# thu-ml/SageAttention

Measured on AMD Instinct MI355X. Metric: attention TFLOPS (causal, hd=128), kernel-only, as published by the reference, higher is better.
Workload: dtype int8 QK^T + fp8(e4m3) PV, fp32 accumulate

## Files before the change

sageattention_amd/csrc/sage_attn.hip:

```cpp
#include "sage_common.h"
#include "sage_kernels.h"
#include "sage_attn_parts.h"
#include "sage_work_order.h"
#include <cstdlib>

#ifndef SAGE_ORDER_DEFAULT
#define SAGE_ORDER_DEFAULT -1
#endif

namespace sage {

static int g_work_order = -2;
int work_order()
{
    if (g_work_order == -2) {
        const char *e = getenv("SAGE_ORDER_GROUP");
        g_work_order = (e != nullptr && e[0] != 0) ? atoi(e) : SAGE_ORDER_DEFAULT;
    }
    return g_work_order;
}
void set_work_order_mode(int group) { g_work_order = group; }

static int plan_grid(AttnParams &q, const AttnVariant &v)
{
    q.order_group = 0;
    q.order_fold = 0;
    q.order_left = 0;
    const int nheads = q.B * q.Hq;
    if (q.cu_q != nullptr && q.work_items != nullptr)
        return 8 * ((q.Hq & 7) * ((q.items_bound + 7) / 8) + (q.Hq >> 3) * q.items_bound);
    if (q.cu_q != nullptr) return ((q.B * q.Hkv + 7) / 8) * 8 * q.group * q.nqblk;
    const int forced = work_order();
    if (!v.causal || v.mask_kind != 0 || v.seeded || q.kv_split > 1 || q.nqblk <= 1 || forced == 0) return nheads * q.nqblk;
    WorkOrder w;
    const int grid = plan_work_order(w, nheads, q.nqblk, q.Lk, v.head_dim, v.pv_fp8, forced);
    q.order_group = w.group;
    q.order_fold = w.fold;
    q.order_left = w.left;
    return grid;
}

static bool route_exists(const AttnParams &p, const AttnVariant &v, const AttnLaunchOpts &o)
{
    const bool varlen = p.cu_q != nullptr, per_thread = v.qf == 1 || v.qf == 2, per_block = v.qf == 3 || v.qf == 4;
    if ((v.head_dim != 64 && v.head_dim != 128) || v.qf < 0 || v.qf > 4 || v.mask_kind < 0 || v.mask_kind > 3) return false;
    if (v.mask_kind != 0 && (v.qf != 0 || v.pv_fp8 || v.causal || v.kthread || !v.two_level)) return false;
    if (per_thread && (varlen || !v.kthread || v.two_level != v.pv_fp8)) return false;
    if (per_block && (v.kthread || (v.pv_fp8 ? (!varlen || o.fp8_folded) : !v.two_level))) return false;
    if (p.v_rows != 0 && (v.pv_fp8 || v.mask_kind != 0 || varlen || p.kv_split > 1 || v.qf == 2 || v.qf == 4)) return false;
    if ((v.seeded || v.kv_lens) && (!per_thread || !v.pv_fp8 || o.fp8_folded || (v.seeded && v.kv_lens))) return false;
    if (v.seeded != (p.seed_max != nullptr) || (v.seeded && p.kv_split < 1)) return false;
    if (v.kv_lens && (p.cu_k == nullptr || p.kv_split > 1)) return false;
    if (v.q_start != (!varlen && p.cu_qs != nullptr) || (v.q_start && (!v.kv_lens || !v.causal))) return false;
    return true;
}

hipError_t launch_attention(const AttnParams &p_in, const AttnVariant &v, const AttnLaunchOpts &o)
{
    AttnParams p = p_in;
    const int nwork = plan_grid(p, v);
    if (o.grid_out != nullptr) *o.grid_out = 0;
    if (nwork <= 0) return hipSuccess;
    if (!route_exists(p, v, o)) return hipErrorInvalidValue;
    const bool d128 = v.head_dim == 128;
    if (v.seeded) return d128 ? launch_attn_f8_seeded<128>(p, v, nwork, o) : launch_attn_f8_seeded<64>(p, v, nwork, o);
    if (v.q_start) return d128 ? launch_attn_f8_qstart<128>(p, v, nwork, o) : launch_attn_f8_qstart<64>(p, v, nwork, o);
    if (v.kv_lens) return d128 ? launch_attn_f8_kvlens<128>(p, v, nwork, o) : launch_attn_f8_kvlens<64>(p, v, nwork, o);
    if (v.pv_fp8 && v.qf >= 3) return d128 ? launch_attn_f8_varlen<128>(p, v, nwork, o) : launch_attn_f8_varlen<64>(p, v, nwork, o);
    if (!v.pv_fp8) return d128 ? launch_attn_part<128, false, true>(p, v, nwork, o) : launch_attn_part<64, false, true>(p, v, nwork, o);
    if (o.fp8_folded) return d128 ? launch_attn_part<128, true, true>(p, v, nwork, o) : launch_attn_part<64, true, true>(p, v, nwork, o);
    return d128 ? launch_attn_part<128, true, false>(p, v, nwork, o) : launch_attn_part<64, true, false>(p, v, nwork, o);
}

}
```

sageattention_amd/csrc/sage_attn_kernel.h:

```cpp
#pragma once
#include "sage_common.h"
#include "sage_kernels.h"
#include "sage_attn_parts.h"
#include "sage_quant_math.h"
#include "sage_work_order.h"
#include <atomic>
#include <climits>
#include <cstdlib>
#include <type_traits>

#ifndef SAGE_ABL
#define SAGE_ABL 0
#endif
#ifndef SAGE_DIAG_PIPE
#define SAGE_DIAG_PIPE 1
#endif
#ifndef SAGE_KARG_PREFETCH
#define SAGE_KARG_PREFETCH 1
#endif
#ifndef SAGE_TAIL_PIPE
#define SAGE_TAIL_PIPE 1
#endif
#ifndef SAGE_KSEL
#define SAGE_KSEL 1
// ... 38 lines not shown
{
    v16i d;
    asm("s_nop 1\n\tv_mfma_i32_32x32x32_i8 %0, %1, %2, 0x3e22f983" : "=&v"(d) : "v"(a), "v"(b));
    return d;
}

#if SAGE_ATTN_TRACE
#define SAGE_TSTAMP(i) do { if (wave == 0) { unsigned long long t_; \
    asm volatile("s_memrealtime %0\n\ts_waitcnt lgkmcnt(0)" : "=s"(t_) :: "memory"); ttrace[i] = (unsigned)t_; } } while (0)
#else
#define SAGE_TSTAMP(i) do { } while (0)
#endif

template <int D, bool PV_FP8, bool CAUSAL, bool KTHREAD, bool TWO_LEVEL, int NH, int MASK = 0, int QF = 0, bool SFOLD = true, bool CPERS = false,
          bool VROWS = false, bool SEED = false, bool QSTART = false, bool KVLEN = false>
__global__ void __launch_bounds__(256, SAGE_MIN_WAVES(D, MASK))
sage_attn_kernel(const AttnParams p_arg)
{
    typedef const __attribute__((address_space(4))) AttnParams *kparams_t;
    const kparams_t kp0 = (kparams_t)__builtin_amdgcn_kernarg_segment_ptr();
    const __attribute__((address_space(4))) AttnParams &p = *kp0;
    (void)p_arg;
#if SAGE_KARG_PREFETCH
    static_assert(sizeof(AttnParams) > 0x180, "prefetch offsets lie inside the parameter block");
    {
        unsigned t0, t1, t2, t3, t4, t5, t6;
        asm volatile("s_load_dword %0, %7, 0x0\n\ts_load_dword %1, %7, 0x40\n\ts_load_dword %2, %7, 0x80\n\ts_load_dword %3, %7, 0xc0\n\t"
                     "s_load_dword %4, %7, 0x100\n\ts_load_dword %5, %7, 0x140\n\ts_load_dword %6, %7, 0x180\n\ts_waitcnt lgkmcnt(0)"
                     : "=&s"(t0), "=&s"(t1), "=&s"(t2), "=&s"(t3), "=&s"(t4), "=&s"(t5), "=&s"(t6) : "s"(kp0) : "memory");
    }
#endif
    using C = TileCfg<D, PV_FP8, NH>;
    constexpr int KT = C::KT;
    constexpr int NS = 2 * NH;
    static_assert(!SEED || (PV_FP8 && KTHREAD && TWO_LEVEL && !SFOLD && MASK == 0 && (QF == 1 || QF == 2) && !CPERS && !VROWS),
                  "the seeded split: FP8 PV, fused per-thread Q, exact score form, dense");
    static_assert(!KVLEN || (PV_FP8 && KTHREAD && TWO_LEVEL && !SFOLD && MASK == 0 && (QF == 1 || QF == 2) && !CPERS && !VROWS && !SEED),
                  "per-sample key lengths: FP8 PV, fused per-thread Q, exact score form, dense");
    static_assert(!QSTART || (KVLEN && CAUSAL), "per-sample query offsets: the causal kv_lens kernels");
    extern __shared__ __attribute__((aligned(16))) unsigned char smem[];

    const int wave_s = __builtin_amdgcn_readfirstlane((int)threadIdx.x >> 6);
#if SAGE_ATTN_TRACE
    __shared__ unsigned ttrace[16];
#endif
    constexpr bool PERS_OK = (!CAUSAL || CPERS) && MASK == 0;
    const bool pers = PERS_OK && p.sched != nullptr;
    __shared__ int s_ticket[2];
    int tpar = 0;
    int bid = blockIdx.x;
    unsigned next_k_v = 0;
    bool have_next = false, own_empty = false;
// ... 38 lines not shown
            if (lane_o == 0) kv = __hip_atomic_fetch_add(sched + 32 * bq, 1u, __ATOMIC_RELAXED, __HIP_MEMORY_SCOPE_AGENT);
            const int i = 32 * ((int)__builtin_amdgcn_readfirstlane(kv) + sched_first) + 8 * (bq & 3) + (bq >> 2);
            if (i < nwg_l) return i;
        }
        return -1;
    };
    while (bid >= 0) {
    next_k_v = 0;
    do {
    kparams_t kp = kp0;
    if constexpr (PERS_OK) asm volatile("" : "+s"(kp));
    const __attribute__((address_space(4))) AttnParams &p = *kp;
    int lane_v = (int)__builtin_amdgcn_mbcnt_hi(~0u, __builtin_amdgcn_mbcnt_lo(~0u, 0u));
    if constexpr (PERS_OK) asm volatile("v_mbcnt_lo_u32_b32 %0, -1, 0\n\tv_mbcnt_hi_u32_b32 %0, -1, %0" : "=v"(lane_v));
    const int lane = lane_v;
    const int wave = wave_s;
    [[maybe_unused]] const int tid = wave * 64 + lane;
    int n = lane & 31;
    int g = lane >> 5;
    SAGE_TSTAMP(0);
    __builtin_amdgcn_s_setreg(kHwregModeFp16Ovfl, 1);

    const int nqblk = p.nqblk;
    int b, h, hk, qblk;
    if (p.cu_q != nullptr && p.work_items != nullptr) {
        typedef const __attribute__((address_space(4))) int *cint_p;
        const cint_p hdr = (cint_p)p.work_hdr;
        const int nitems = hdr[0];
        const WorkOrder wo = {hdr[1], hdr[2], hdr[3]};
        const int nwg = 8 * (wo.left * ((nitems + 7) >> 3) + (p.Hq >> 3) * nitems);
        int qrank;
        if (bid >= nwg || !work_item(wo, bid, nwg, p.Hq, nitems, h, qrank)) break;
        const cint_p items = (cint_p)p.work_items;
        b = items[2 * qrank];
        qblk = items[2 * qrank + 1];
        hk = h / p.group;
    } else if (p.cu_q != nullptr) {
        const int xcd = bid & 7, idx = bid >> 3;
        const int per_unit = nqblk * p.group;
        const int j = idx / per_unit, within = idx - j * per_unit;
        const int u = j * 8 + xcd;
        if (u >= p.B * p.Hkv) break;
        const int r = within / p.group, hg = within - r * p.group;
        qblk = nqblk - 1 - r;
        const int bs = u / p.Hkv;
        hk = u - bs * p.Hkv;
        b = p.seq_order != nullptr ? p.seq_order[bs] : bs;
        h = hk * p.group + hg;
    } else {
        int bh, qrank;
        const WorkOrder wo = {CAUSAL ? p.order_group : 0, p.order_fold, p.order_left};
        if (!work_item(wo, bid, pers ? p.nwg : (int)gridDim.x, p.B * p.Hq, nqblk, bh, qrank)) break;
        qblk = nqblk - 1 - qrank;
        b = bh / p.Hq;
        h = bh - b * p.Hq;
        hk = h / p.group;
    }

    int Lq = p.Lq, Lk = p.Lk;
    [[maybe_unused]] int qstart = 0;
    long q_off, k_off, o_off;
    long v_tile0, v_tstride;
    const float *qs_ptr, *ks_ptr;
    int qs_stride, ks_tstride;
    if (p.cu_q != nullptr) {
        typedef const __attribute__((address_space(4))) int *cint_p;
        const int bu = __builtin_amdgcn_readfirstlane(b);
        const int q0 = ((cint_p)p.cu_q)[bu], k0 = ((cint_p)p.cu_k)[bu], q1 = ((cint_p)p.cu_q)[bu + 1], k1 = ((cint_p)p.cu_k)[bu + 1];
        const int ks0 = ((cint_p)p.cu_ks)[bu];
        Lq = q1 - q0;
        Lk = k1 - k0;
        if (qblk * BLKQ >= Lq) break;
        q_off = (long)q0 * p.q_sl + (long)h * p.q_sh;
        k_off = (long)k0 * p.k_sl + (long)hk * p.k_sh;
        o_off = (long)q0 * p.o_sl + (long)h * p.o_sh;
        v_tile0 = (long)ks0 * p.Hkv + hk;
        v_tstride = p.Hkv;
        qs_ptr = QF == 0 ? p.q_scale + ((long)((cint_p)p.cu_qs)[bu] + qblk) * p.Hq + h : nullptr;
        qs_stride = 0;
        ks_ptr = p.k_scale + (long)ks0 * p.Hkv + hk;
        ks_tstride = p.Hkv;
    } else if constexpr (SEED) {
        const int hk0 = hk / p.kv_split, kc0 = p.kv_base + (hk - hk0 * p.kv_split) * Lk;
        const long bh0 = (long)b * (p.Hkv / p.kv_split) + hk0;
        q_off = (long)b * p.q_sb + (long)(hk0 * p.group + (h - hk * p.group)) * p.q_sh;
        k_off = (long)b * p.k_sb + (long)hk0 * p.k_sh + (long)kc0 * p.k_sl;
        o_off = (long)b * p.o_sb + (long)h * p.o_sh;
        v_tile0 = bh0 * (p.nks >> 2) + (kc0 >> 6);
        v_tstride = 1;
        qs_ptr = nullptr;
        qs_stride = 0;
        ks_ptr = p.k_scale + bh0 * p.nks + (kc0 >> 6) * 4;
        ks_tstride = 4;
    } else {
        const int hq = p.kv_split > 1 ? (hk / p.kv_split) * p.group + (h - hk * p.group) : h;
        if constexpr (KVLEN) {
            typedef const __attribute__((address_space(4))) int *cint_p;
            const int len = ((cint_p)p.cu_k)[__builtin_amdgcn_readfirstlane(b)];
            Lk = len < 0 ? 0 : (len < p.Lk ? len : p.Lk);
            if constexpr (QSTART) {
                const int s = ((cint_p)p.cu_qs)[__builtin_amdgcn_readfirstlane(b)];
                qstart = s < -p.Lq ? -p.Lq : (s < p.Lk ? s : p.Lk);
            }
        }
        q_off = (long)b * p.q_sb + (long)hq * p.q_sh;
        k_off = (long)b * p.k_sb + (long)hk * p.k_sh;
        o_off = (long)b * p.o_sb + (long)h * p.o_sh;
        const int ntk = ((KVLEN ? p.Lk : Lk) + BLKK - 1) / BLKK;
        v_tile0 = ((long)b * p.Hkv + hk) * ntk;
        v_tstride = 1;
        qs_ptr = p.q_scale + ((long)b * p.Hq + h) * p.nqs + (long)qblk * p.qs_per_blk;
        qs_stride = 1;
        ks_ptr = p.k_scale + ((long)b * p.Hkv + hk) * p.nks;
        ks_tstride = KTHREAD ? 4 : 1;
    }

    SAGE_TSTAMP(1);
    const int row0 = qblk * BLKQ + wave * 32;
    int my_row = row0 + n;
    const int kchunk0 = QSTART ? -qstart
                      : SEED ? (CAUSAL ? p.kv_base + (hk % p.kv_split) * Lk : 0)
                             : ((CAUSAL && p.kv_split > 1 && p.cu_q == nullptr) ? (hk % p.kv_split) * Lk : 0);
    const int crow0 = row0 - kchunk0;
    int cmy_row = my_row - kchunk0;
    const int ntk_all = (Lk + BLKK - 1) / BLKK;
    int n_iters = (Lk + KT - 1) / KT;
    if (CAUSAL) {
        int lim = (qblk * BLKQ + BLKQ - kchunk0 + KT - 1) / KT;
        lim = lim > 0 ? lim : 0;
        n_iters = lim < n_iters ? lim : n_iters;
    }

    v4i qf[C::KSTEPS];
    float qsc;
    const unsigned char *kbase = reinterpret_cast<const unsigned char *>(p.k) + k_off;
    static_assert(!VROWS || (!PV_FP8 && MASK == 0), "V rows in place: FP16 PV, unmasked, dense launches");
    const unsigned char *vbase = reinterpret_cast<const unsigned char *>(p.v) + (VROWS ? 2 * ((long)b * p.v_sb + (long)hk * p.v_sh) : 0L);
    constexpr int CPR = D / 16;
    constexpr int KP = C::K_TILE_BYTES / 1024, VP = C::V_IMG_BYTES / 1024;
    unsigned koff[KP / 4];
#pragma unroll
    for (int i = 0; i < KP / 4; i++) {
        const int e = (wave * (KP / 4) + i) * 64 + lane;
        const int row = e / CPR, phys = e % CPR;
        koff[i] = (unsigned)(row * (int)p.k_sl + swz_chunk<D>(row, phys) * 16);
// ... 168 lines not shown
        amax = fmaxf(amax, __shfl_xor(amax, 32));
        if constexpr (QBLOCK) {
            __shared__ float q_amax[4];
            if (lane == 0) q_amax[wave] = amax;
            asm volatile("s_waitcnt lgkmcnt(0)" ::: "memory");
            __builtin_amdgcn_s_barrier();
            amax = fmaxf(fmaxf(q_amax[0], q_amax[1]), fmaxf(q_amax[2], q_amax[3]));
        }
        const float sc = quant_scale(amax, QBLOCK ? QS_TRITON : QS_TRITON_THREAD);
        const float y = quant_recip(sc);
        qsc = sc;
#pragma unroll
        for (int ks = 0; ks < C::KSTEPS; ks++) {
            int q8[16];
#pragma unroll
            for (int j = 0; j < 16; j++) q8[j] = QBLOCK ? quant_round_triton(x[ks][j], sc, y) : quant_round_triton_nz(x[ks][j], sc, y);
#pragma unroll
            for (int w = 0; w < 4; w++) qf[ks][w] = (int)pack_int8x4(q8[4 * w], q8[4 * w + 1], q8[4 * w + 2], q8[4 * w + 3]);
        }
    }

    if constexpr (SEED) {
        if (my_row < Lq) {
            const int hk0 = hk / p.kv_split;
            const long gl = (long)p.group * Lq;
            const float *sm = p.seed_max + ((long)b * (p.Hkv / p.kv_split) + hk0) * p.seed_chunks * gl + (long)(h - hk * p.group) * Lq + my_row;
            const int c_end = p.seed_first + (hk - hk0 * p.kv_split);
            for (int c = 0; c < c_end; c++) m_run = fmaxf(m_run, sm[c * gl]);
        }
    }
    SAGE_TSTAMP(2);
    ring_wait(n_iters > 1);
    SAGE_TSTAMP(3);

    int cur = 0;
    auto tile_iter = [&](const int it) {
        const bool more = (it + 1) < n_iters;
        const bool more2 = (it + 2) < n_iters;
        const int nxt = (cur + 1 == NSTAGE) ? 0 : cur + 1;
        float ksc_next[NH][2];
        if (more) load_kscales(it + 1, ksc_next);
        if (more2) issue_loads(it + 2, (nxt + 1 == NSTAGE) ? 0 : nxt + 1);

        int nact = 0;
#pragma unroll
        for (int hh = 0; hh < NH; hh++) {
            const int key0 = it * KT + hh * BLKK;
            if (key0 < Lk && (!CAUSAL || key0 <= crow0 + 31)) nact = hh + 1;
        }
// ... 247 lines not shown
        }
    }
    if constexpr (MASK == 0) {
        asm volatile("v_mbcnt_lo_u32_b32 %0, -1, 0\n\tv_mbcnt_hi_u32_b32 %0, -1, %0" : "=v"(lane_g));
        n = lane_g & 31;
        g = lane_g >> 5;
        my_row = row0 + n;
        cmy_row = my_row - kchunk0;
    }
#pragma nounroll
    for (; it < n_iters; it++) tile_iter(it);
    SAGE_TSTAMP(4);
    __syncthreads();
    SAGE_TSTAMP(5);
    if (pers && !own_empty) {
        if (wave == 0 && lane_g == 0) next_k_v = __hip_atomic_fetch_add(kpl()->sched + 32 * my_queue(), 1u, __ATOMIC_RELAXED, __HIP_MEMORY_SCOPE_AGENT);
        have_next = true;
    }

    __builtin_amdgcn_s_setreg(kHwregModeFp16Ovfl, 0);
    const float l_tot = pair_sum(l_run);
    const float inv = l_tot > 0.0f ? __builtin_amdgcn_rcpf(l_tot) : 0.0f;
    if (p.lse != nullptr && g == 0 && my_row < Lq) {
        long lidx = (p.cu_q != nullptr) ? ((long)h * p.lse_sh + p.cu_q[b] + my_row)
                                        : ((long)b * p.Hq + h) * (long)p.Lq + my_row;
        p.lse[lidx] = __builtin_amdgcn_logf(l_tot) + m_run;
    }
    unsigned char *obuf = smem + wave * (32 * D * 2);
    const long vbh = SEED ? (long)b * (p.Hkv / p.kv_split) + hk / p.kv_split : (long)b * p.Hkv + hk;
    const float *vsc = PV_FP8 ? p.v_scale + vbh * D : nullptr;
    const float *vmn = (p.v_mean != nullptr) ? p.v_mean + vbh * D : nullptr;
    v4f sc4[C::DT][4], mn4[C::DT][4];
    [[maybe_unused]] unsigned keep = (!KVLEN || Lk > 0) ? ~0u : 0u;
    if constexpr (KVLEN) asm volatile("" : "+v"(keep));
#pragma unroll
    for (int dt = 0; dt < C::DT; dt++) {
#pragma unroll
        for (int r4 = 0; r4 < 4; r4++) {
            const v4f one = {1.0f, 1.0f, 1.0f, 1.0f};
            sc4[dt][r4] = PV_FP8 ? *reinterpret_cast<const v4f *>(vsc + dt * 32 + 8 * r4 + 4 * g) : one;
        }
        if (vmn != nullptr) {
#pragma unroll
            for (int r4 = 0; r4 < 4; r4++) mn4[dt][r4] = *reinterpret_cast<const v4f *>(vmn + dt * 32 + 8 * r4 + 4 * g);
        } else {
#pragma unroll
            for (int r4 = 0; r4 < 4; r4++) { const v4f z = {0.0f, 0.0f, 0.0f, 0.0f}; mn4[dt][r4] = z; }
        }
    }
#pragma unroll
    for (int dt = 0; dt < C::DT; dt++) {
#pragma unroll
        for (int r4 = 0; r4 < 4; r4++) {
            const int d0 = dt * 32 + 8 * r4 + 4 * g;
            float x[4];
#pragma unroll
            for (int j = 0; j < 4; j++) {
                x[j] = o[dt][4 * r4 + j] * inv;
                if (PV_FP8) x[j] *= sc4[dt][r4][j];
                if constexpr (KVLEN) x[j] = __uint_as_float(__float_as_uint(x[j]) & keep);
                x[j] += mn4[dt][r4][j];
            }
            if constexpr (SEED) {
                if (my_row < Lq) *reinterpret_cast<v4f *>(reinterpret_cast<float *>(p.o) + o_off + (long)my_row * p.o_sl + d0) = v4f{x[0], x[1], x[2], x[3]};
                continue;
            }
            v2u pk;
            if (p.out_dtype == DT_F16) {
                pk[0] = (unsigned)f32_to_f16_rne(x[0]) | ((unsigned)f32_to_f16_rne(x[1]) << 16);
                pk[1] = (unsigned)f32_to_f16_rne(x[2]) | ((unsigned)f32_to_f16_rne(x[3]) << 16);
            } else {
                pk[0] = (unsigned)f32_to_bf16_rne(x[0]) | ((unsigned)f32_to_bf16_rne(x[1]) << 16);
                pk[1] = (unsigned)f32_to_bf16_rne(x[2]) | ((unsigned)f32_to_bf16_rne(x[3]) << 16);
            }
            const int q8 = d0 >> 2;
            const int Q = (q8 >> 1) ^ (n & 7);
            *reinterpret_cast<v2u *>(obuf + n * (D * 2) + Q * 16 + (q8 & 1) * 8) = pk;
        }
    }
    asm volatile("s_waitcnt lgkmcnt(0)" ::: "memory");
    if constexpr (!SEED) {
        constexpr int LPR = D * 2 / 16;
        constexpr int RPP = 64 / LPR;
        unsigned char *obase = reinterpret_cast<unsigned char *>(p.o) + 2 * o_off;
#pragma unroll
        for (int pass = 0; pass < 32 / RPP; pass++) {
            const int r = pass * RPP + lane_g / LPR, Q = lane_g % LPR;
            const v4u val = *reinterpret_cast<const v4u *>(obuf + r * (D * 2) + (Q ^ (r & 7)) * 16);
            const int grow = row0 + r;
            if (grow < Lq) *reinterpret_cast<v4u *>(obase + 2 * ((long)grow * p.o_sl) + Q * 16) = val;
        }
    }
#if SAGE_ATTN_TRACE
    SAGE_TSTAMP(6);
    asm volatile("s_waitcnt vmcnt(0)" ::: "memory");
    SAGE_TSTAMP(7);
    if (wave == 0 && p.trace != nullptr && bid < p.trace_wgs) {
        if (lane < 8 || lane == 8 || lane >= 13) p.trace[16 * bid + lane] = ttrace[lane];
        if (lane == 9) p.trace[16 * bid + 9] = __builtin_amdgcn_s_getreg((31 << 11) | 4);
        if (lane == 10) p.trace[16 * bid + 10] = __builtin_amdgcn_s_getreg((31 << 11) | 20);
        if (lane == 11) p.trace[16 * bid + 11] = blockIdx.x;
        if (lane == 12) p.trace[16 * bid + 12] = (unsigned)qblk;
    }
#endif
    } while (0);
    if (!pers) break;
    if (wave_s == 0) { const int t = resolve_ticket(); if (__builtin_amdgcn_mbcnt_hi(~0u, __builtin_amdgcn_mbcnt_lo(~0u, 0u)) == 0) s_ticket[tpar] = t; }
    __syncthreads();
    bid = __builtin_amdgcn_readfirstlane(s_ticket[tpar]);
    tpar ^= 1;
    }
    if constexpr (PERS_OK) {
        if (pers && wave_s == 0) {
// ... 14 lines not shown
```

sageattention_amd/csrc/sage_cabi.hip:

```cpp
#include "../../include/sage_gfx950.h"
#include "sage_common.h"
#include "sage_kernels.h"
#include "sage_work_order.h"

#include <cstdarg>
#include <cstddef>
#include <cstdio>
#include <cstdlib>
#include <cstring>

namespace {

thread_local char g_err[512] = "";

int fail(int code, const char *fmt, ...)
{
    va_list ap;
    va_start(ap, fmt);
    vsnprintf(g_err, sizeof(g_err), fmt, ap);
    va_end(ap);
    return code;
}

inline bool aligned16(const void *p) { return (reinterpret_cast<uintptr_t>(p) & 15u) == 0; }
// ... 186 lines not shown
                        c.kv_lens != nullptr ? "sage_attn_fused_q_pv_f8_kvlens launch" : "sage_attn_fused_q launch");
}

}

extern "C" {

SAGE_API int sage_abi_version(void) { return SAGE_ABI_VERSION; }
SAGE_API const char *sage_last_error(void) { return g_err; }
SAGE_API int sage_debug_work_order_plan(int nheads, int nqblk, int64_t kv_len, int head_dim, int pv_fp8, int forced, int *group, int *fold, int *left)
{
    if (nheads <= 0 || nqblk <= 0 || group == nullptr || fold == nullptr || left == nullptr) return fail(SAGE_EINVAL, "sage_debug_work_order_plan: bad argument");
    sage::WorkOrder w;
    const int grid = sage::plan_work_order(w, nheads, nqblk, (long)kv_len, head_dim, pv_fp8 != 0, forced);
    *group = w.group; *fold = w.fold; *left = w.left;
    return grid;
}
SAGE_API int sage_debug_work_item(int bid, int nwg, int nheads, int nqblk, int group, int fold, int left, int *head, int *qrank)
{
    if (head == nullptr || qrank == nullptr || nwg <= 0 || bid < 0 || bid >= nwg || nheads <= 0 || nqblk <= 0 || group < 0 || fold < 0 || fold > 1 ||
        left < 0 || left >= 8 || left > nheads)
        return fail(SAGE_EINVAL, "sage_debug_work_item: bad argument");
    const sage::WorkOrder w = {group, fold, left};
    return sage::work_item(w, bid, nwg, nheads, nqblk, *head, *qrank) ? 1 : 0;
}
SAGE_API int sage_work_order(void) { return sage::work_order(); }
SAGE_API void sage_set_work_order(int group) { sage::set_work_order_mode(group < -1 ? -1 : group); }

SAGE_API int64_t sage_v_image_bytes(int head_dim, int fp8, int64_t n_kv_tiles_total)
{
    return n_kv_tiles_total * (int64_t)head_dim * (fp8 ? 64 : 128);
}

static int quant_common(const void *x, const void *mean, int8_t *out, float *scale,
                        int B, int H, int L, int D,
                        int64_t x_sb, int64_t x_sh, int64_t x_sl,
                        int64_t o_sb, int64_t o_sh, int64_t o_sl,
                        int64_t mean_sb, int64_t mean_sh,
                        int blk, int warp, int gran, int is_key, int style,
                        float pre_scale, int dtype, void *stream, const int32_t *kv_lens)
{
    SAGE_REQUIRE(x && out && scale, "null tensor pointer");
    SAGE_REQUIRE_HEAD_DIM(D, "");
    SAGE_REQUIRE(blk == 64 || blk == 128, "blk must be 64 or 128 (got %d)", blk);
    SAGE_REQUIRE(B > 0 && H > 0 && L > 0, "empty tensor");
    SAGE_REQUIRE_DTYPE(dtype, "dtype");
    SAGE_REQUIRE(style >= 0 && style <= 2, "bad style %d", style);
// ... 891 lines not shown
```

sageattention_amd/csrc/sage_common.h:

```cpp
#pragma once
#include <hip/hip_runtime.h>
#include <stdint.h>

namespace sage {

typedef int v4i __attribute__((ext_vector_type(4)));
typedef int v8i __attribute__((ext_vector_type(8)));
typedef int v16i __attribute__((ext_vector_type(16)));
typedef float v16f __attribute__((ext_vector_type(16)));
typedef float v4f __attribute__((ext_vector_type(4)));
typedef float v2f __attribute__((ext_vector_type(2)));
typedef _Float16 v8h __attribute__((ext_vector_type(8)));
typedef _Float16 v2h __attribute__((ext_vector_type(2)));
typedef unsigned int v4u __attribute__((ext_vector_type(4)));
typedef unsigned int v2u __attribute__((ext_vector_type(2)));

constexpr int kWave = 64;
constexpr int BLKQ = 128;
constexpr int BLKK = 64;
constexpr float kFp8Offset = 8.807f;
constexpr float kNegBig = -1.0e30f;

enum : int { DT_F16 = 0, DT_BF16 = 1 };

// ... 15 lines not shown
__device__ inline uint16_t f32_to_bf16_rne(float f)
{
    uint32_t x = __float_as_uint(f);
    x += 0x7fffu + ((x >> 16) & 1u);
    return (uint16_t)(x >> 16);
}
__device__ inline float f16_to_f32(uint16_t h)
{
    _Float16 v; __builtin_memcpy(&v, &h, 2); return (float)v;
}
__device__ inline uint16_t f32_to_f16_rne(float f)
{
    _Float16 v = (_Float16)f; uint16_t h; __builtin_memcpy(&h, &v, 2); return h;
}
template <int DT> __device__ inline float ld16(uint16_t raw)
{
    if constexpr (DT == DT_F16) return f16_to_f32(raw); else return bf16_to_f32(raw);
}
template <int DT> __device__ inline uint16_t st16(float f)
{
    if constexpr (DT == DT_F16) return f32_to_f16_rne(f); else return f32_to_bf16_rne(f);
}

__device__ inline float pair_max(float x)
{
    auto r = __builtin_amdgcn_permlane32_swap(__float_as_uint(x), __float_as_uint(x), false, false);
    return fmaxf(__uint_as_float(r[0]), __uint_as_float(r[1]));
}
__device__ inline float pair_sum(float x)
{
    auto r = __builtin_amdgcn_permlane32_swap(__float_as_uint(x), __float_as_uint(x), false, false);
    return __uint_as_float(r[0]) + __uint_as_float(r[1]);
}

template <typename IntPtr>
__device__ __forceinline__ void varlen_segment(IntPtr cu, int nseq, int total, int seg, int &t0, int &len)
{
    if (seg < nseq) { t0 = cu[seg]; len = cu[seg + 1] - t0; }
    else if (seg == nseq) { t0 = cu[nseq]; len = total - t0; }
    else { t0 = 0; len = cu[0]; }
    len = len > 0 ? len : 0;
}

}
```

sageattention_amd/csrc/sage_kernels.h:

```cpp
#pragma once
#include <hip/hip_runtime.h>
#include <stdint.h>

namespace sage {

enum : int { QG_PER_BLOCK = 1, QG_PER_WARP32 = 2, QG_PER_THREAD = 3, QG_PER_WARP16 = 4, QG_PER_THREAD16 = 5 };

constexpr int kAttnSchedBytes = 32 * 128;
constexpr int kAttnSchedDoneWord = 16;

struct AttnParams {
    const void *q;
    const int8_t *k;
    const void *v;
    long v_sb, v_sh, v_sl;
    int v_rows;
    void *o;
    float *lse;
    const float *q_scale;
    const float *k_scale;
    const float *v_scale;
    const float *v_mean;
    const void *mask;
    long m_sb, m_sh, m_sq, m_sk;
    const int32_t *cu_q;
// ... 9 lines not shown
    int B, Hq, Hkv, group;
    int Lq, Lk;
    int nqblk;
    long q_sb, q_sh, q_sl;
    long k_sb, k_sh, k_sl;
    long o_sb, o_sh, o_sl;
    int nqs, nks;
    int qs_per_blk;
    int q_gran;
    int kv_split;
    int ks_shift;
    int out_dtype;
    long lse_sh;
    float sm_scale_log2;
    float q_premul;
    int order_group;
    int order_fold;
    int order_left;
    unsigned *trace;
    int trace_wgs;
    const float *seed_max;
    int seed_chunks, seed_first;
    int kv_base;
};

struct AttnLaunchOpts {
    hipStream_t stream;
    bool fp8_folded;
    bool force_persistent;
    int *grid_out;
};
struct AttnVariant {
    int head_dim;
    bool pv_fp8;
    bool causal;
    bool kthread;
    bool two_level;
    int mask_kind;
    int qf;
    bool seeded;
    bool kv_lens;
    bool q_start;
};
constexpr int attn_qf(bool per_block, int q_dtype) { return (per_block ? 3 : 1) + (q_dtype == 0 ? 0 : 1); }
hipError_t launch_attention(const AttnParams &p, const AttnVariant &v, const AttnLaunchOpts &o);

// ... 165 lines not shown
```

sageattention_amd/csrc/sage_work_order.h:

```cpp
#pragma once

#if defined(__HIPCC__)
#define SAGE_HD __host__ __device__ __forceinline__
#else
#define SAGE_HD inline
#endif

namespace sage {

struct WorkOrder {
    int group;
    int fold;
    int left;
};

SAGE_HD bool work_item(const WorkOrder &w, int bid, int nwg, int nheads, int nqblk, int &head, int &qrank)
{
    const int xcd = bid & 7, idx = bid >> 3;
    const int qq = nwg >> 3, rr = nwg & 7;
    if (w.group <= 0) {
        const int wid = (xcd < rr ? xcd * (qq + 1) : rr * (qq + 1) + (xcd - rr) * qq) + idx;
        head = wid / nqblk;
        qrank = wid - head * nqblk;
        return true;
    }
    int r = idx;
    if (w.fold != 0 && idx >= 32) r = qq - 1 - (idx - 32);
    const int hpx = nheads >> 3;
    const int left_cnt = w.left * ((nqblk + 7) >> 3);
    if (r < left_cnt) {
        const int oct = r / w.left;
        head = r - oct * w.left;
        qrank = 8 * oct + ((oct & 1) ? 7 - xcd : xcd);
        return qrank < nqblk;
    }
    r -= left_cnt;
    const int gsz = w.group * nqblk;
    const int gi = r / gsz, within = r - gi * gsz;
    const int rest = hpx - gi * w.group;
    const int gc = rest < w.group ? rest : w.group;
    qrank = within / gc;
    head = w.left + xcd * hpx + gi * w.group + (within - qrank * gc);
    return true;
}

SAGE_HD int plan_work_order(WorkOrder &w, int nheads, int nqblk, long kv_len, int head_dim, bool pv_fp8, int forced)
{
    const int hpx = nheads / 8, left = nheads % 8;
    const int wg_per_cu = head_dim == 64 ? 3 : 2;
    const int slots = 32 * wg_per_cu;
    const int g_bal = (2 * slots + nqblk) / (nqblk + 1);
    const long head_bytes = kv_len * head_dim * (pv_fp8 ? 2 : 3);
    const int g_l2 = (int)((4L << 20) / (head_bytes > 0 ? head_bytes : 1));
    const int g_more = 2 * g_bal < g_l2 ? 2 * g_bal : g_l2;
    int grp = forced > 0 ? forced : (g_bal > g_more ? g_bal : g_more);
    grp = grp > hpx ? hpx : grp;
    grp = grp < 1 ? 1 : grp;
    w.group = grp;
    w.left = left;
    const int cnt = left * ((nqblk + 7) / 8) + hpx * nqblk;
    const bool one_sorted_list = (left == 0 && grp >= hpx) || hpx == 0;
    w.fold = (wg_per_cu == 2 && cnt > 32 && cnt <= 64 && one_sorted_list) ? 1 : 0;
    return 8 * cnt;
}


// ... 55 lines not shown
```

Before: 1623.

## Precompute fast integer dividers on host and restructure output epilogue

Replaces the runtime integer divisions in the kernel prologue (work-order mapping, head/group/split indices) with multiply-shift dividers computed on the host and passed in the kernel parameters. The parameter block grows, so the kernarg prefetch gains an eighth load. The epilogue is also restructured: normalisation and scale loops are split and gated at compile time, packing uses vector conversions, and the LDS swizzle and global store addressing use precomputed pointers. Debug entry points for checking the fast divide and the pack routine are added.

```diff
diff --git a/sageattention_amd/csrc/sage_attn.hip b/sageattention_amd/csrc/sage_attn.hip
--- a/sageattention_amd/csrc/sage_attn.hip
+++ b/sageattention_amd/csrc/sage_attn.hip
@@ -40,6 +40,18 @@
     return grid;
 }
 
+static void plan_divisions(AttnParams &q)
+{
+    const WorkOrder w = {q.order_group, q.order_fold, q.order_left};
+    q.order_divs = make_work_divs(w, q.B * q.Hq, q.nqblk);
+    q.div_Hq = make_fast_div(q.Hq);
+    q.div_group = make_fast_div(q.group);
+    q.div_Hkv = make_fast_div(q.Hkv);
+    q.div_split = make_fast_div(q.kv_split);
+    q.div_unit = make_fast_div(q.group * q.nqblk);
+    q.hkv_unsplit = q.kv_split >= 1 ? q.Hkv / q.kv_split : q.Hkv;
+}
+
 static bool route_exists(const AttnParams &p, const AttnVariant &v, const AttnLaunchOpts &o)
 {
     const bool varlen = p.cu_q != nullptr, per_thread = v.qf == 1 || v.qf == 2, per_block = v.qf == 3 || v.qf == 4;
@@ -62,6 +74,7 @@
     if (o.grid_out != nullptr) *o.grid_out = 0;
     if (nwork <= 0) return hipSuccess;
     if (!route_exists(p, v, o)) return hipErrorInvalidValue;
+    plan_divisions(p);
     const bool d128 = v.head_dim == 128;
     if (v.seeded) return d128 ? launch_attn_f8_seeded<128>(p, v, nwork, o) : launch_attn_f8_seeded<64>(p, v, nwork, o);
     if (v.q_start) return d128 ? launch_attn_f8_qstart<128>(p, v, nwork, o) : launch_attn_f8_qstart<64>(p, v, nwork, o);
diff --git a/sageattention_amd/csrc/sage_attn_kernel.h b/sageattention_amd/csrc/sage_attn_kernel.h
--- a/sageattention_amd/csrc/sage_attn_kernel.h
+++ b/sageattention_amd/csrc/sage_attn_kernel.h
@@ -84,12 +84,13 @@
     const __attribute__((address_space(4))) AttnParams &p = *kp0;
     (void)p_arg;
 #if SAGE_KARG_PREFETCH
-    static_assert(sizeof(AttnParams) > 0x180, "prefetch offsets lie inside the parameter block");
+    static_assert(sizeof(AttnParams) > 0x1c0 && sizeof(AttnParams) <= 0x200, "prefetch offsets cover the parameter block, and lie inside it");
     {
-        unsigned t0, t1, t2, t3, t4, t5, t6;
-        asm volatile("s_load_dword %0, %7, 0x0\n\ts_load_dword %1, %7, 0x40\n\ts_load_dword %2, %7, 0x80\n\ts_load_dword %3, %7, 0xc0\n\t"
-                     "s_load_dword %4, %7, 0x100\n\ts_load_dword %5, %7, 0x140\n\ts_load_dword %6, %7, 0x180\n\ts_waitcnt lgkmcnt(0)"
-                     : "=&s"(t0), "=&s"(t1), "=&s"(t2), "=&s"(t3), "=&s"(t4), "=&s"(t5), "=&s"(t6) : "s"(kp0) : "memory");
+        unsigned t0, t1, t2, t3, t4, t5, t6, t7;
+        asm volatile("s_load_dword %0, %8, 0x0\n\ts_load_dword %1, %8, 0x40\n\ts_load_dword %2, %8, 0x80\n\ts_load_dword %3, %8, 0xc0\n\t"
+                     "s_load_dword %4, %8, 0x100\n\ts_load_dword %5, %8, 0x140\n\ts_load_dword %6, %8, 0x180\n\ts_load_dword %7, %8, 0x1c0\n\t"
+                     "s_waitcnt lgkmcnt(0)"
+                     : "=&s"(t0), "=&s"(t1), "=&s"(t2), "=&s"(t3), "=&s"(t4), "=&s"(t5), "=&s"(t6), "=&s"(t7) : "s"(kp0) : "memory");
     }
 #endif
     using C = TileCfg<D, PV_FP8, NH>;
@@ -174,6 +175,7 @@
     __builtin_amdgcn_s_setreg(kHwregModeFp16Ovfl, 1);
 
     const int nqblk = p.nqblk;
+    auto kdiv = [](const __attribute__((address_space(4))) FastDiv &f) -> FastDiv { return FastDiv{f.mul, f.shift}; };
     int b, h, hk, qblk;
     if (p.cu_q != nullptr && p.work_items != nullptr) {
         typedef const __attribute__((address_space(4))) int *cint_p;
@@ -182,31 +184,32 @@
         const WorkOrder wo = {hdr[1], hdr[2], hdr[3]};
         const int nwg = 8 * (wo.left * ((nitems + 7) >> 3) + (p.Hq >> 3) * nitems);
         int qrank;
-        if (bid >= nwg || !work_item(wo, bid, nwg, p.Hq, nitems, h, qrank)) break;
+        if (bid >= nwg || !work_item(wo, WorkDivide{}, bid, nwg, p.Hq, nitems, h, qrank)) break;
         const cint_p items = (cint_p)p.work_items;
         b = items[2 * qrank];
         qblk = items[2 * qrank + 1];
-        hk = h / p.group;
+        hk = fast_div(h, kdiv(p.div_group));
     } else if (p.cu_q != nullptr) {
         const int xcd = bid & 7, idx = bid >> 3;
         const int per_unit = nqblk * p.group;
-        const int j = idx / per_unit, within = idx - j * per_unit;
+        const int j = fast_div(idx, kdiv(p.div_unit)), within = idx - j * per_unit;
         const int u = j * 8 + xcd;
         if (u >= p.B * p.Hkv) break;
-        const int r = within / p.group, hg = within - r * p.group;
+        const int r = fast_div(within, kdiv(p.div_group)), hg = within - r * p.group;
         qblk = nqblk - 1 - r;
-        const int bs = u / p.Hkv;
+        const int bs = fast_div(u, kdiv(p.div_Hkv));
         hk = u - bs * p.Hkv;
         b = p.seq_order != nullptr ? p.seq_order[bs] : bs;
         h = hk * p.group + hg;
     } else {
         int bh, qrank;
         const WorkOrder wo = {CAUSAL ? p.order_group : 0, p.order_fold, p.order_left};
-        if (!work_item(wo, bid, pers ? p.nwg : (int)gridDim.x, p.B * p.Hq, nqblk, bh, qrank)) break;
+        const WorkDivs dv = {kdiv(p.order_divs.nqblk), kdiv(p.order_divs.left), kdiv(p.order_divs.gsz), kdiv(p.order_divs.gc_full), kdiv(p.order_divs.gc_last)};
+        if (!work_item(wo, dv, bid, pers ? p.nwg : (int)gridDim.x, p.B * p.Hq, nqblk, bh, qrank)) break;
         qblk = nqblk - 1 - qrank;
-        b = bh / p.Hq;
+        b = fast_div(bh, kdiv(p.div_Hq));
         h = bh - b * p.Hq;
-        hk = h / p.group;
+        hk = fast_div(h, kdiv(p.div_group));
     }
 
     int Lq = p.Lq, Lk = p.Lk;
@@ -233,8 +236,8 @@
         ks_ptr = p.k_scale + (long)ks0 * p.Hkv + hk;
         ks_tstride = p.Hkv;
     } else if constexpr (SEED) {
-        const int hk0 = hk / p.kv_split, kc0 = p.kv_base + (hk - hk0 * p.kv_split) * Lk;
-        const long bh0 = (long)b * (p.Hkv / p.kv_split) + hk0;
+        const int hk0 = fast_div(hk, kdiv(p.div_split)), kc0 = p.kv_base + (hk - hk0 * p.kv_split) * Lk;
+        const long bh0 = (long)b * p.hkv_unsplit + hk0;
         q_off = (long)b * p.q_sb + (long)(hk0 * p.group + (h - hk * p.group)) * p.q_sh;
         k_off = (long)b * p.k_sb + (long)hk0 * p.k_sh + (long)kc0 * p.k_sl;
         o_off = (long)b * p.o_sb + (long)h * p.o_sh;
@@ -245,7 +248,7 @@
         ks_ptr = p.k_scale + bh0 * p.nks + (kc0 >> 6) * 4;
         ks_tstride = 4;
     } else {
-        const int hq = p.kv_split > 1 ? (hk / p.kv_split) * p.group + (h - hk * p.group) : h;
+        const int hq = p.kv_split > 1 ? fast_div(hk, kdiv(p.div_split)) * p.group + (h - hk * p.group) : h;
         if constexpr (KVLEN) {
             typedef const __attribute__((address_space(4))) int *cint_p;
             const int len = ((cint_p)p.cu_k)[__builtin_amdgcn_readfirstlane(b)];
@@ -270,9 +273,10 @@
     SAGE_TSTAMP(1);
     const int row0 = qblk * BLKQ + wave * 32;
     int my_row = row0 + n;
+    [[maybe_unused]] const int chunk = hk - fast_div(hk, kdiv(p.div_split)) * p.kv_split;
     const int kchunk0 = QSTART ? -qstart
-                      : SEED ? (CAUSAL ? p.kv_base + (hk % p.kv_split) * Lk : 0)
-                             : ((CAUSAL && p.kv_split > 1 && p.cu_q == nullptr) ? (hk % p.kv_split) * Lk : 0);
+                      : SEED ? (CAUSAL ? p.kv_base + chunk * Lk : 0)
+                             : ((CAUSAL && p.kv_split > 1 && p.cu_q == nullptr) ? chunk * Lk : 0);
     const int crow0 = row0 - kchunk0;
     int cmy_row = my_row - kchunk0;
     const int ntk_all = (Lk + BLKK - 1) / BLKK;
@@ -487,9 +491,9 @@
 
     if constexpr (SEED) {
         if (my_row < Lq) {
-            const int hk0 = hk / p.kv_split;
+            const int hk0 = fast_div(hk, kdiv(p.div_split));
             const long gl = (long)p.group * Lq;
-            const float *sm = p.seed_max + ((long)b * (p.Hkv / p.kv_split) + hk0) * p.seed_chunks * gl + (long)(h - hk * p.group) * Lq + my_row;
+            const float *sm = p.seed_max + ((long)b * p.hkv_unsplit + hk0) * p.seed_chunks * gl + (long)(h - hk * p.group) * Lq + my_row;
             const int c_end = p.seed_first + (hk - hk0 * p.kv_split);
             for (int c = 0; c < c_end; c++) m_run = fmaxf(m_run, sm[c * gl]);
         }
@@ -783,73 +787,118 @@
     const float l_tot = pair_sum(l_run);
     const float inv = l_tot > 0.0f ? __builtin_amdgcn_rcpf(l_tot) : 0.0f;
     if (p.lse != nullptr && g == 0 && my_row < Lq) {
-        long lidx = (p.cu_q != nullptr) ? ((long)h * p.lse_sh + p.cu_q[b] + my_row)
-                                        : ((long)b * p.Hq + h) * (long)p.Lq + my_row;
-        p.lse[lidx] = __builtin_amdgcn_logf(l_tot) + m_run;
-    }
-    unsigned char *obuf = smem + wave * (32 * D * 2);
-    const long vbh = SEED ? (long)b * (p.Hkv / p.kv_split) + hk / p.kv_split : (long)b * p.Hkv + hk;
+        typedef const __attribute__((address_space(4))) int *cint_p;
+        long lhead = (p.cu_q != nullptr) ? ((long)h * p.lse_sh + ((cint_p)p.cu_q)[__builtin_amdgcn_readfirstlane(b)]) : ((long)b * p.Hq + h) * (long)p.Lq;
+        asm volatile("" : "+s"(lhead));
+        p.lse[lhead + my_row] = __builtin_amdgcn_logf(l_tot) + m_run;
+    }
+    const long vbh = SEED ? (long)b * p.hkv_unsplit + fast_div(hk, kdiv(p.div_split)) : (long)b * p.Hkv + hk;
     const float *vsc = PV_FP8 ? p.v_scale + vbh * D : nullptr;
     const float *vmn = (p.v_mean != nullptr) ? p.v_mean + vbh * D : nullptr;
-    v4f sc4[C::DT][4], mn4[C::DT][4];
+    [[maybe_unused]] v4f sc4[C::DT][4];
     [[maybe_unused]] unsigned keep = (!KVLEN || Lk > 0) ? ~0u : 0u;
     if constexpr (KVLEN) asm volatile("" : "+v"(keep));
-#pragma unroll
-    for (int dt = 0; dt < C::DT; dt++) {
-#pragma unroll
-        for (int r4 = 0; r4 < 4; r4++) {
-            const v4f one = {1.0f, 1.0f, 1.0f, 1.0f};
-            sc4[dt][r4] = PV_FP8 ? *reinterpret_cast<const v4f *>(vsc + dt * 32 + 8 * r4 + 4 * g) : one;
-        }
-        if (vmn != nullptr) {
-#pragma unroll
-            for (int r4 = 0; r4 < 4; r4++) mn4[dt][r4] = *reinterpret_cast<const v4f *>(vmn + dt * 32 + 8 * r4 + 4 * g);
+    if constexpr (PV_FP8) {
+#pragma unroll
+        for (int dt = 0; dt < C::DT; dt++)
+#pragma unroll
+            for (int r4 = 0; r4 < 4; r4++) sc4[dt][r4] = *reinterpret_cast<const v4f *>(vsc + dt * 32 + 8 * r4 + 4 * g);
+    }
+    [[maybe_unused]] long o_row_bytes = 2 * (long)p.o_sl;
+    typedef __attribute__((address_space(1))) unsigned char *global_bytes;
+    [[maybe_unused]] global_bytes o_tile = (global_bytes)p.o + 2 * o_off;
+    if constexpr (!SEED) asm volatile("" : "+s"(o_row_bytes), "+s"(o_tile));
+    __builtin_amdgcn_sched_barrier(0);
+    if constexpr (PV_FP8) {
+#pragma unroll
+        for (int dt = 0; dt < C::DT; dt++)
+#pragma unroll
+            for (int i = 0; i < 16; i++) o[dt][i] *= inv;
+    }
+    __builtin_amdgcn_sched_barrier(0);
+    if constexpr (KVLEN) {
+#pragma unroll
+        for (int dt = 0; dt < C::DT; dt++)
+#pragma unroll
+            for (int i = 0; i < 16; i++) o[dt][i] = __uint_as_float(__float_as_uint(o[dt][i] * sc4[dt][i >> 2][i & 3]) & keep);
+        __builtin_amdgcn_sched_barrier(0);
+    }
+    auto scale_o = [&](auto mean_tag) {
+        constexpr bool MEAN = decltype(mean_tag)::value;
+        [[maybe_unused]] v4f mn4[C::DT][4];
+        if constexpr (MEAN) {
+#pragma unroll
+            for (int dt = 0; dt < C::DT; dt++)
+#pragma unroll
+                for (int r4 = 0; r4 < 4; r4++) mn4[dt][r4] = *reinterpret_cast<const v4f *>(vmn + dt * 32 + 8 * r4 + 4 * g);
+            __builtin_amdgcn_sched_barrier(0);
+        }
+#pragma unroll
+        for (int dt = 0; dt < C::DT; dt++)
+#pragma unroll
+            for (int r4 = 0; r4 < 4; r4++)
+#pragma unroll
+                for (int j = 0; j < 4; j++) {
+                    float x = o[dt][4 * r4 + j];
+                    if constexpr (KVLEN) { }
+                    else if constexpr (PV_FP8) x *= sc4[dt][r4][j];
+                    else x *= inv;
+                    if constexpr (MEAN) x += mn4[dt][r4][j];
+                    else x += 0.0f;
+                    o[dt][4 * r4 + j] = x;
+                }
+    };
+    if (vmn != nullptr) scale_o(std::true_type{});
+    else scale_o(std::false_type{});
+    if constexpr (SEED) {
+        if (my_row < Lq) {
+            float *orow = reinterpret_cast<float *>(p.o) + o_off + (long)my_row * p.o_sl + 4 * g;
+#pragma unroll
+            for (int dt = 0; dt < C::DT; dt++)
+#pragma unroll
+                for (int r4 = 0; r4 < 4; r4++)
+                    *reinterpret_cast<v4f *>(orow + dt * 32 + 8 * r4) = v4f{o[dt][4 * r4], o[dt][4 * r4 + 1], o[dt][4 * r4 + 2], o[dt][4 * r4 + 3]};
+        }
+    } else {
+        unsigned pk[C::DT][8];
+        if (p.out_dtype == DT_F16) {
+#pragma unroll
+            for (int dt = 0; dt < C::DT; dt++)
+#pragma unroll
+                for (int i = 0; i < 8; i++) pk[dt][i] = pack2_16<DT_F16>(o[dt][2 * i], o[dt][2 * i + 1]);
         } else {
 #pragma unroll
-            for (int r4 = 0; r4 < 4; r4++) { const v4f z = {0.0f, 0.0f, 0.0f, 0.0f}; mn4[dt][r4] = z; }
-        }
-    }
-#pragma unroll
-    for (int dt = 0; dt < C::DT; dt++) {
-#pragma unroll
-        for (int r4 = 0; r4 < 4; r4++) {
-            const int d0 = dt * 32 + 8 * r4 + 4 * g;
-            float x[4];
-#pragma unroll
-            for (int j = 0; j < 4; j++) {
-                x[j] = o[dt][4 * r4 + j] * inv;
-                if (PV_FP8) x[j] *= sc4[dt][r4][j];
-                if constexpr (KVLEN) x[j] = __uint_as_float(__float_as_uint(x[j]) & keep);
-                x[j] += mn4[dt][r4][j];
-            }
-            if constexpr (SEED) {
-                if (my_row < Lq) *reinterpret_cast<v4f *>(reinterpret_cast<float *>(p.o) + o_off + (long)my_row * p.o_sl + d0) = v4f{x[0], x[1], x[2], x[3]};
-                continue;
-            }
-            v2u pk;
-            if (p.out_dtype == DT_F16) {
-                pk[0] = (unsigned)f32_to_f16_rne(x[0]) | ((unsigned)f32_to_f16_rne(x[1]) << 16);
-                pk[1] = (unsigned)f32_to_f16_rne(x[2]) | ((unsigned)f32_to_f16_rne(x[3]) << 16);
-            } else {
-                pk[0] = (unsigned)f32_to_bf16_rne(x[0]) | ((unsigned)f32_to_bf16_rne(x[1]) << 16);
-                pk[1] = (unsigned)f32_to_bf16_rne(x[2]) | ((unsigned)f32_to_bf16_rne(x[3]) << 16);
-            }
-            const int q8 = d0 >> 2;
-            const int Q = (q8 >> 1) ^ (n & 7);
-            *reinterpret_cast<v2u *>(obuf + n * (D * 2) + Q * 16 + (q8 & 1) * 8) = pk;
-        }
-    }
-    asm volatile("s_waitcnt lgkmcnt(0)" ::: "memory");
-    if constexpr (!SEED) {
-        constexpr int LPR = D * 2 / 16;
+            for (int dt = 0; dt < C::DT; dt++)
+#pragma unroll
+                for (int i = 0; i < 8; i++) pk[dt][i] = pack2_16<DT_BF16>(o[dt][2 * i], o[dt][2 * i + 1]);
+        }
+        constexpr int ROWB = D * 2;
+        typedef __attribute__((address_space(3))) v2u *lds_v2u;
+        typedef __attribute__((address_space(3))) const v4u *lds_cv4u;
+        const unsigned region = (unsigned)wave * (32 * ROWB);
+        const unsigned wlane = region + (unsigned)(n * ROWB + 8 * g + 16 * (n & 7));
+#pragma unroll
+        for (int dt = 0; dt < C::DT; dt++)
+#pragma unroll
+            for (int r4 = 0; r4 < 4; r4++) {
+                const int c = 4 * dt + r4;
+                *(lds_v2u)((lds_bytes)smem + (wlane ^ (unsigned)(16 * (c & 7))) + 128 * (c >> 3)) = v2u{pk[dt][2 * r4], pk[dt][2 * r4 + 1]};
+            }
+        asm volatile("s_waitcnt lgkmcnt(0)" ::: "memory");
+        constexpr int LPR = ROWB / 16;
         constexpr int RPP = 64 / LPR;
-        unsigned char *obase = reinterpret_cast<unsigned char *>(p.o) + 2 * o_off;
+        static_assert(RPP == 4 || RPP == 8, "the read swizzle below splits into a lane part and a pass part");
+        const int rl = (int)((unsigned)lane_g / LPR), Q = (int)((unsigned)lane_g % LPR);
+        const unsigned rlane = region + (unsigned)(rl * ROWB + 16 * (Q ^ rl));
+        global_bytes optr = o_tile + (long)row0 * o_row_bytes + 16 * Q;
+#pragma unroll
+        for (int bit = 0; (1 << bit) < RPP; bit++) optr += ((rl >> bit) & 1) ? (o_row_bytes << bit) : 0L;
+        const int rows_left = Lq - row0 - rl;
 #pragma unroll
         for (int pass = 0; pass < 32 / RPP; pass++) {
-            const int r = pass * RPP + lane_g / LPR, Q = lane_g % LPR;
-            const v4u val = *reinterpret_cast<const v4u *>(obuf + r * (D * 2) + (Q ^ (r & 7)) * 16);
-            const int grow = row0 + r;
-            if (grow < Lq) *reinterpret_cast<v4u *>(obase + 2 * ((long)grow * p.o_sl) + Q * 16) = val;
+            const v4u val = *(lds_cv4u)((lds_bytes)smem + (rlane ^ (unsigned)(16 * ((pass * RPP) & 7))) + pass * RPP * ROWB);
+            if (pass * RPP < rows_left) *(__attribute__((address_space(1))) v4u *)optr = val;
+            optr += RPP * o_row_bytes;
         }
     }
 #if SAGE_ATTN_TRACE
diff --git a/sageattention_amd/csrc/sage_cabi.hip b/sageattention_amd/csrc/sage_cabi.hip
--- a/sageattention_amd/csrc/sage_cabi.hip
+++ b/sageattention_amd/csrc/sage_cabi.hip
@@ -232,7 +232,58 @@
         left < 0 || left >= 8 || left > nheads)
         return fail(SAGE_EINVAL, "sage_debug_work_item: bad argument");
     const sage::WorkOrder w = {group, fold, left};
-    return sage::work_item(w, bid, nwg, nheads, nqblk, *head, *qrank) ? 1 : 0;
+    return sage::work_item(w, sage::make_work_divs(w, nheads, nqblk), bid, nwg, nheads, nqblk, *head, *qrank) ? 1 : 0;
+}
+
+SAGE_API int sage_debug_fast_div(int n, int d) { return sage::fast_div(n, sage::make_fast_div(d)); }
+SAGE_API long long sage_debug_fast_div_sweep(int d_lo, int d_hi, int n_max, int *bad_n, int *bad_d)
+{
+    long long bad = 0;
+    for (long long d = d_lo < 1 ? 1 : d_lo; d <= d_hi; d++) {
+        const sage::FastDiv f = sage::make_fast_div((int)d);
+        auto check = [&](unsigned n) {
+            if (n > 0x7fffffffu || sage::fast_div((int)n, f) == (int)(n / (unsigned)d)) return;
+            if (bad++ == 0) { if (bad_n != nullptr) *bad_n = (int)n; if (bad_d != nullptr) *bad_d = (int)d; }
+        };
+        for (long long n = 0; n <= n_max; n++) check((unsigned)n);
+        for (unsigned k = 0; k < 64; k++) check(0x7fffffffu - k);
+        for (unsigned k = 0; k < 32; k++) { check((1u << k) - 1u); check(1u << k); check((1u << k) + 1u); }
+        for (unsigned k = 1; k <= 64; k++) { check((unsigned)(0x7fffffffu / (unsigned)d / k * (unsigned)d)); check((unsigned)(0x7fffffffu / (unsigned)d / k * (unsigned)d) - 1u); }
+    }
+    return bad;
+}
+SAGE_API int sage_debug_work_divs_check(int nwg, int nheads, int nqblk, int group, int fold, int left)
+{
+    if (nwg <= 0 || nheads <= 0 || nqblk <= 0 || group < 0 || left < 0 || left >= 8) return fail(SAGE_EINVAL, "sage_debug_work_divs_check: bad argument");
+    const sage::WorkOrder w = {group, fold, left};
+    const sage::WorkDivs dv = sage::make_work_divs(w, nheads, nqblk);
+    int bad = 0;
+    for (int bid = 0; bid < nwg; bid++) {
+        int h0 = -1, r0 = -1, h1 = -1, r1 = -1;
+        const bool a = sage::work_item(w, dv, bid, nwg, nheads, nqblk, h0, r0), b = sage::work_item(w, bid, nwg, nheads, nqblk, h1, r1);
+        bad += (a != b || h0 != h1 || r0 != r1) ? 1 : 0;
+    }
+    return bad;
+}
+}
+
+namespace {
+template <int DT> __global__ void debug_pack2_16_kernel(const float *x, unsigned *out, int npairs)
+{
+    const int i = blockIdx.x * blockDim.x + threadIdx.x;
+    if (i < npairs) out[i] = sage::pack2_16<DT>(x[2 * i], x[2 * i + 1]);
+}
+}
+
+extern "C" {
+SAGE_API int sage_debug_pack2_16(const float *x, void *out, int npairs, int dtype, void *stream)
+{
+    SAGE_REQUIRE(x != nullptr && out != nullptr && npairs > 0, "sage_debug_pack2_16: bad argument");
+    SAGE_REQUIRE_DTYPE(dtype, "dtype");
+    const dim3 grid((npairs + 255) / 256), block(256);
+    if (dtype == SAGE_DTYPE_F16) hipLaunchKernelGGL(debug_pack2_16_kernel<sage::DT_F16>, grid, block, 0, static_cast<hipStream_t>(stream), x, static_cast<unsigned *>(out), npairs);
+    else hipLaunchKernelGGL(debug_pack2_16_kernel<sage::DT_BF16>, grid, block, 0, static_cast<hipStream_t>(stream), x, static_cast<unsigned *>(out), npairs);
+    return check_launch(hipGetLastError(), "sage_debug_pack2_16");
 }
 SAGE_API int sage_work_order(void) { return sage::work_order(); }
 SAGE_API void sage_set_work_order(int group) { sage::set_work_order_mode(group < -1 ? -1 : group); }
diff --git a/sageattention_amd/csrc/sage_common.h b/sageattention_amd/csrc/sage_common.h
--- a/sageattention_amd/csrc/sage_common.h
+++ b/sageattention_amd/csrc/sage_common.h
@@ -61,6 +61,17 @@
     if constexpr (DT == DT_F16) return f32_to_f16_rne(f); else return f32_to_bf16_rne(f);
 }
 
+template <int DT> __device__ __forceinline__ unsigned pack2_16(float a, float b)
+{
+    const v2f x = {a, b};
+    if constexpr (DT == DT_F16) {
+        return __builtin_bit_cast(unsigned, __builtin_convertvector(x, v2h));
+    } else {
+        typedef __bf16 v2bf __attribute__((ext_vector_type(2)));
+        return __builtin_bit_cast(unsigned, __builtin_convertvector(x, v2bf));
+    }
+}
+
 __device__ inline float pair_max(float x)
 {
     auto r = __builtin_amdgcn_permlane32_swap(__float_as_uint(x), __float_as_uint(x), false, false);
diff --git a/sageattention_amd/csrc/sage_kernels.h b/sageattention_amd/csrc/sage_kernels.h
--- a/sageattention_amd/csrc/sage_kernels.h
+++ b/sageattention_amd/csrc/sage_kernels.h
@@ -1,6 +1,7 @@
 #pragma once
 #include <hip/hip_runtime.h>
 #include <stdint.h>
+#include "sage_work_order.h"
 
 namespace sage {
 
@@ -56,6 +57,10 @@
     const float *seed_max;
     int seed_chunks, seed_first;
     int kv_base;
+    WorkDivs order_divs;
+    FastDiv div_Hq, div_group, div_Hkv, div_split;
+    FastDiv div_unit;
+    int hkv_unsplit;
 };
 
 struct AttnLaunchOpts {
diff --git a/sageattention_amd/csrc/sage_work_order.h b/sageattention_amd/csrc/sage_work_order.h
--- a/sageattention_amd/csrc/sage_work_order.h
+++ b/sageattention_amd/csrc/sage_work_order.h
@@ -14,13 +14,54 @@
     int left;
 };
 
-SAGE_HD bool work_item(const WorkOrder &w, int bid, int nwg, int nheads, int nqblk, int &head, int &qrank)
+struct FastDiv {
+    unsigned mul, shift;
+};
+SAGE_HD FastDiv make_fast_div(int d)
+{
+    FastDiv f = {0u, 0u};
+    if (d <= 0) return f;
+    while (f.shift < 31u && (1u << f.shift) < (unsigned)d) f.shift++;
+    f.mul = (unsigned)((((unsigned long long)1 << (31u + f.shift)) + (unsigned)d - 1u) / (unsigned)d);
+    return f;
+}
+SAGE_HD int fast_div(int n, const FastDiv &f)
+{
+    return (int)((unsigned)(((unsigned long long)((unsigned)n << 1) * f.mul) >> 32) >> f.shift);
+}
+
+struct WorkDivs {
+    FastDiv nqblk, left, gsz, gc_full, gc_last;
+    SAGE_HD int by_nqblk(int n, int) const { return fast_div(n, nqblk); }
+    SAGE_HD int by_left(int n, int) const { return fast_div(n, left); }
+    SAGE_HD int by_gsz(int n, int) const { return fast_div(n, gsz); }
+    SAGE_HD int by_gc(int n, int gc, int group) const { return fast_div(n, gc == group ? gc_full : gc_last); }
+};
+struct WorkDivide {
+    SAGE_HD int by_nqblk(int n, int d) const { return n / d; }
+    SAGE_HD int by_left(int n, int d) const { return n / d; }
+    SAGE_HD int by_gsz(int n, int d) const { return n / d; }
+    SAGE_HD int by_gc(int n, int gc, int) const { return n / gc; }
+};
+SAGE_HD WorkDivs make_work_divs(const WorkOrder &w, int nheads, int nqblk)
+{
+    WorkDivs d;
+    d.nqblk = make_fast_div(nqblk);
+    d.left = make_fast_div(w.left);
+    d.gsz = make_fast_div(w.group > 0 ? w.group * nqblk : 0);
+    d.gc_full = make_fast_div(w.group);
+    d.gc_last = make_fast_div(w.group > 0 ? (nheads >> 3) % w.group : 0);
+    return d;
+}
+
+template <class Div>
+SAGE_HD bool work_item(const WorkOrder &w, const Div &dv, int bid, int nwg, int nheads, int nqblk, int &head, int &qrank)
 {
     const int xcd = bid & 7, idx = bid >> 3;
     const int qq = nwg >> 3, rr = nwg & 7;
     if (w.group <= 0) {
         const int wid = (xcd < rr ? xcd * (qq + 1) : rr * (qq + 1) + (xcd - rr) * qq) + idx;
-        head = wid / nqblk;
+        head = dv.by_nqblk(wid, nqblk);
         qrank = wid - head * nqblk;
         return true;
     }
@@ -29,19 +70,23 @@
     const int hpx = nheads >> 3;
     const int left_cnt = w.left * ((nqblk + 7) >> 3);
     if (r < left_cnt) {
-        const int oct = r / w.left;
+        const int oct = dv.by_left(r, w.left);
         head = r - oct * w.left;
         qrank = 8 * oct + ((oct & 1) ? 7 - xcd : xcd);
         return qrank < nqblk;
     }
     r -= left_cnt;
     const int gsz = w.group * nqblk;
-    const int gi = r / gsz, within = r - gi * gsz;
+    const int gi = dv.by_gsz(r, gsz), within = r - gi * gsz;
     const int rest = hpx - gi * w.group;
     const int gc = rest < w.group ? rest : w.group;
-    qrank = within / gc;
+    qrank = dv.by_gc(within, gc, w.group);
     head = w.left + xcd * hpx + gi * w.group + (within - qrank * gc);
     return true;
+}
+SAGE_HD bool work_item(const WorkOrder &w, int bid, int nwg, int nheads, int nqblk, int &head, int &qrank)
+{
+    return work_item(w, WorkDivide{}, bid, nwg, nheads, nqblk, head, qrank);
 }
 
 SAGE_HD int plan_work_order(WorkOrder &w, int nheads, int nqblk, long kv_len, int head_dim, bool pv_fp8, int forced)
```

After: 1636 (median of 6 runs). Within noise of the previous version (+0.8%).
